# sdroh1027/DiffusionVID

Measured on AMD Instinct MI355X. Metric: frames/sec (1000x600) DiffusionVID-R101 x1, higher is better.
Workload: dtype f16

## Files before the change

### diffusionvid_amd/csrc/kernels.h

```cpp
#pragma once
#include "common.h"

struct IgemmParams {
    const half_t* in;
    const half_t* w;
    const float* bias;
    const void* res;
    void* out;
    int H, W, Cin, Ho, Wo, Cout, KH, KW, stride, pad;
    int M, Kpad, ntaps, ldc, alg_k;
    int relu, out_f32, res_mode, res_f32;
    int splitk;
    long split_stride;
    int tiles_m, tiles_n;
};
int dvid_igemm_launch(const IgemmParams& p, hipStream_t s);
int dvid_igemm2_launch(const IgemmParams& p, hipStream_t s);

bool dvid_conv3x3_halo_supported(const IgemmParams& p);
bool dvid_conv3x3_halo_preferred(const IgemmParams& p);
int dvid_conv3x3_halo_launch(const IgemmParams& p, hipStream_t s);
bool dvid_stem_pool_supported(const IgemmParams& p);
int dvid_stem_pool_launch(const IgemmParams& p, hipStream_t s);

bool dvid_wstat_supported(const IgemmParams& p);
bool dvid_wstat_preferred(const IgemmParams& p);
int dvid_wstat_launch(const IgemmParams& p, hipStream_t s);

bool dvid_bneck64_tail_preferred(int H, int W);
int dvid_bneck128_tail_launch(const half_t* t1, const half_t* w2, const float* b2, const half_t* w3, const float* b3, const half_t* res,
                              const half_t* w1n, const float* b1n, half_t* out, half_t* t1n, int n, int H, int W, hipStream_t s);
int dvid_bneck64_tail_launch(const half_t* t1, const half_t* w2, const float* b2, const half_t* w3, const float* b3, const half_t* res,
                             const half_t* ws, const float* bs, const half_t* w1n, const float* b1n, int n_next, half_t* out, half_t* t1n,
                             int n, int H, int W, hipStream_t s);

struct FrameTable {
    static constexpr int kMax = 32;
    const float* p[kMax];
};
int dvid_prep_images_launch(const float* const* frames, half_t* nhwc8, int n, int h, int w, const float* mean, const float* inv_std,
                            hipStream_t s);
int dvid_prep_images_s2d_launch(const float* const* frames, half_t* s2d16, int n, int h, int w, const float* mean, const float* inv_std,
                                hipStream_t s);
int dvid_maxpool3x3s2_launch(const half_t* in, half_t* out, int n, int h, int w, int c, hipStream_t s);
int dvid_nchw_from_nhwc_launch(const half_t* in, float* out, int n, int h, int w, int c, hipStream_t s);
int dvid_nhwc_from_nchw_launch(const float* in, half_t* out, int n, int h, int w, int c, hipStream_t s);
int dvid_add_layernorm_launch(const float* x, const float* r, const float* g, const float* b, float* y32, half_t* y16,
                              int rows, int d, int relu, hipStream_t s, int nsplit = 1, long split_stride = 0,
                              const float* xbias = nullptr);
int dvid_f32_to_f16_launch(const float* x, half_t* y, long n, hipStream_t s);
int dvid_resize_u8_launch(const unsigned char* src, int h, int w, unsigned char* tmp, float* out, int oh, int ow, int ph, int pw,
                          const int* xbounds, const int* xk, int xksize, const int* ybounds, const int* yk, int yksize, hipStream_t s);
int dvid_modulate_launch(const float* x, const float* scale, int scale_ld, const float* shift, int shift_per_row, int shift_ld,
                         half_t* y16, int rows, int rows_per_frame, int d, hipStream_t s);
int dvid_silu_f16_launch(const float* x, half_t* y, long n, hipStream_t s);

template <typename T>
struct RoiLevelsT {
    const T* feat[3];
    int h[3], w[3];
    float scale[3];
};
using RoiLevels = RoiLevelsT<half_t>;
using RoiLevels32 = RoiLevelsT<float>;
int dvid_roialign_launch(const RoiLevels& lv, int channels, const float* boxes, int n_img, int boxes_per_img, half_t* roi_out,
                         float* mean_out, hipStream_t s);

int dvid_mha_mfma_launch(const half_t* q, const half_t* k, const half_t* v, half_t* out, half_t* vt_scratch, int batch, int lq,
                         int lk, int nheads, int q_ld, int kv_ld, int out_ld, long q_bs, long kv_bs, long out_bs, hipStream_t s);

struct OutProjLnParams {
    const void* x;
    int mode;
    const half_t* wf_hi;
    const half_t* wf_lo;
    const float* w32;
    const float* wscale;
    const float* bias;
    const float* gamma;
    const float* beta;
    float* out;
    int rows, d;
    int* range_flag;
};
int dvid_outproj_ln_launch(const OutProjLnParams& p, hipStream_t s);

constexpr int SWIN_RELBIAS_PITCH = 64;
int dvid_swin_window_attn_launch(const half_t* qkv, const half_t* qkv_bias16, const float* relbias, half_t* out, int batch, int H,
                                 int W, int C, int nheads, int shift, hipStream_t s);
constexpr int SWIN12_RELBIAS_PITCH = 160;
int dvid_swin_window12_attn_launch(const half_t* qkv, const half_t* qkv_bias16, const float* relbias, half_t* out, int batch, int H,
                                   int W, int C, int nheads, int shift, hipStream_t s);
int dvid_patch_merge_ln_launch(const float* x, const float* g, const float* b, half_t* y16, int B, int H, int W, int C, hipStream_t s,
                               float* y32 = nullptr);

int dvid_dynconv_launch(const half_t* roi, const half_t* params, const float* g1, const float* b1, const float* g2,
                        const float* b2, half_t* out, int rows, hipStream_t s);
int dvid_dynconv_roi_launch(const RoiLevels& lv, int channels, const float* boxes, int n_img, int boxes_per_img, const half_t* params,
                            const float* g1, const float* b1, const float* g2, const float* b2, half_t* out, hipStream_t s);

struct HeadTailParams {
    const half_t* x16;
    const float* obj32;
    const half_t* w1f;
    const float* b1;
    const half_t* w2f;
    const float* b2;
    const float* n3g;
    const float* n3b;
    const float* scale;
    int ss_stride, rows_per_frame;
    const float* cond32;
    const half_t* wcf;
    const float* bc;
    int num_cls, num_reg, num_classes, dff;
    const half_t* clsf[4];
    const float* clsg[4];
    const float* clsb[4];
    const half_t* regf[4];
    const float* regg[4];
    const float* regb[4];
    const half_t* wlogf;
    const float* blog;
    const half_t* wdelf;
    const float* bdel;
    const float* boxes;
    float* obj_out;
    float* logits;
    float* boxes_out;
    int* bad_flag;
    long R;
    float wx, wy, ww, wh, clamp;
};
bool dvid_head_tail_supported(int hidden, int dff, int num_cls, int num_reg, int num_classes);
int dvid_head_tail_launch(const HeadTailParams& p, hipStream_t s);

int dvid_apply_deltas_launch(const float* deltas, int delta_ld, const float* boxes, float* out, int n, float wx, float wy, float ww,
                             float wh, float clamp, int* bad_flag, hipStream_t s);
int dvid_counter_normal_launch(float* out, long per_image, int n_images, uint64_t key0, hipStream_t s);
int dvid_noise_to_boxes_launch(const float* x, float* boxes, int n, float scale, float w, float h, hipStream_t s);
int dvid_topk_mask_launch(const float* logits, int n_img, int m, int c, int k1, int k2, const float* feats, int d, float* out1,
                          float* out2, hipStream_t s);

int dvid_ddim_renew_launch(const float* logits, const float* boxes, const float* xt, const float* noise, const float* fresh,
                           float* out, int n_img, int m, int c, float w, float h, float scale, float sra, float srm1, float sqrt_an,
                           float cc, float sigma, float thr, hipStream_t s);

int dvid_topk_candidates_launch(const float* logits, const float* boxes, int n_img, int nsets, int m, int c, float* cand_boxes,
                                float* cand_scores, int* cand_labels, hipStream_t s);
int dvid_topk_stream_launch(const float* logits, const float* boxes, int n_img, int nsets, int m, int c, float* cand_boxes,
                            float* cand_scores, int* cand_labels, hipStream_t s);
int dvid_nms_frames_launch(const float* cand_boxes, const float* cand_scores, const int* cand_labels, int n_img, int n, float img_w,
                           float img_h, float iou, int use_nms, int out_cap, float* out_boxes, float* out_scores, int* out_labels,
                           int* out_counts, hipStream_t s);
bool dvid_nms_frames_fits_lds(int n);
size_t dvid_nms_tiled_scratch_size(int n_img, int n);
int dvid_nms_frames_tiled_launch(const float* cand_boxes, const float* cand_scores, const int* cand_labels, int n_img, int n, float img_w,
                                 float img_h, float iou, int use_nms, int out_cap, float* out_boxes, float* out_scores, int* out_labels,
                                 int* out_counts, void* scratch, hipStream_t s);

long long dvid_seq_nms_scratch_size(const int* class_counts, const int* video_starts, int n_videos, int num_classes);
int dvid_seq_nms_launch(const float* dets, const int* counts, const int* class_counts, const int* video_starts, int n_videos, int cap, int num_classes,
                        unsigned char* keep, float* scores, int* status, void* scratch, hipStream_t s);

int dvid_cdist_launch(const float* x, int n, int d, float* dist, hipStream_t s);
int dvid_fps_launch(const float* dist, int n, int m, int bs_emul, int* idx, hipStream_t s);
int dvid_gather_rows_launch(const float* x, const int* idx, float* y, int m, int d, hipStream_t s);

struct F32GemmParams {
    const float* in;
    const float* w;
    const half_t* w_hi;
    const half_t* w_lo;
    const float* bias;
    int* range_flag;
    const float* wscale;
    const float* res;
    float* out;
    int H, W, Cin, Ho, Wo, Cout, KH, KW, stride, pad;
    int M, K, Kpad, ldc;
    int relu, res_mode;
    int tiles_m, tiles_n;
};
int dvid_f32_igemm_launch(const F32GemmParams& p, hipStream_t s);
bool dvid_f32_wstat_supported(const F32GemmParams& p);
bool dvid_f32_wstat_preferred(const F32GemmParams& p);
int dvid_f32_wstat_tile_rows(const F32GemmParams& p);
int dvid_f32_wstat_launch_tiles(const F32GemmParams& p, hipStream_t s);
bool dvid_f32_conv3x3_supported(const F32GemmParams& p);
int dvid_f32_conv3x3_launch(const F32GemmParams& p, hipStream_t s);
int dvid_f32_prep_images_launch(const float* const* frames, float* nhwc4, int n, int h, int w, const float* mean, const float* std_, hipStream_t s);
int dvid_f32_maxpool3x3s2_launch(const float* in, float* out, int n, int h, int w, int c, hipStream_t s);
int dvid_f32_silu_launch(const float* x, float* y, long n, hipStream_t s);
int dvid_f32_modulate_launch(const float* x, const float* scale, int scale_ld, const float* shift, int shift_per_row, int shift_ld, float* y,
                             int rows, int rows_per_frame, int d, hipStream_t s);
int dvid_f32_roialign_launch(const RoiLevels32& lv, int channels, const float* boxes, int n_img, int boxes_per_img, float* roi_out,
                             float* mean_out, hipStream_t s);
int dvid_f32_mha_launch(const float* q, const float* k, const float* v, float* out, int batch, int lq, int lk, int nheads, int q_ld, int kv_ld,
                        int out_ld, long q_bs, long kv_bs, long out_bs, hipStream_t s);
int dvid_f32_swin_window_attn_launch(const float* qkv, const float* qkv_bias, const float* relbias, float* out, int batch, int H, int W, int C,
                                     int nheads, int shift, hipStream_t s);
int dvid_f32_swin_window12_attn_launch(const float* qkv, const float* qkv_bias, const float* relbias, float* out, int batch, int H, int W, int C,
                                       int nheads, int shift, hipStream_t s);
int dvid_f32_dynconv_launch(const float* roi, const float* params, const float* g1, const float* b1, const float* g2, const float* b2,
                            float* out, int rows, int* range_flag, hipStream_t s);
```

### diffusionvid_amd/csrc/profile.hip

```cpp
#include <mutex>

#include "runtime.h"

bool g_prof_on = false;

namespace {
std::mutex g_prof_mu;
std::vector<ProfRec> g_prof;
std::vector<ProfRec> g_prof_pool;

int prof_take(ProfRec* r) {
    std::lock_guard<std::mutex> lock(g_prof_mu);
    if (!g_prof_pool.empty()) {
        r->a = g_prof_pool.back().a;
        r->b = g_prof_pool.back().b;
        g_prof_pool.pop_back();
        return DVID_OK;
    }
    HIP_TRY(hipEventCreate(&r->a));
    HIP_TRY(hipEventCreate(&r->b));
    return DVID_OK;
}
}

int prof_begin(ProfRec* r, hipStream_t s) {
    if (prof_take(r) != DVID_OK) return DVID_ERR_HIP;
    HIP_TRY(hipEventRecord(r->a, s));
    return DVID_OK;
}
int prof_end(const ProfRec& r, hipStream_t s) {
    HIP_TRY(hipEventRecord(r.b, s));
    std::lock_guard<std::mutex> lock(g_prof_mu);
    g_prof.push_back(r);
    return DVID_OK;
}

int igemm(const IgemmParams& p, hipStream_t s) {
    if (!g_prof_on) return dvid_igemm_launch(p, s);
    ProfRec r{.M = p.M, .N = p.Cout, .K = p.Kpad, .taps = p.ntaps, .stride = p.stride, .res_mode = p.res_mode, .family = true};
    r.flop = 2.0 * p.M * (double)p.Cout * (double)p.alg_k;
    const double in_px = (double)p.M * (p.ntaps > 1 ? p.stride * p.stride : 1);
    r.bytes = in_px * p.Cin * 2.0 + (double)p.Cout * p.Kpad * 2.0 +
              (double)p.M * p.Cout * (p.out_f32 ? 4.0 : 2.0) * (p.splitk > 1 ? p.splitk : 1) +
              (p.res_mode == 1 ? (double)p.M * p.Cout * (p.res_f32 ? 4.0 : 2.0) : p.res_mode == 2 ? (double)p.M * p.Cout * 0.5 : 0.0);
    r.kind = dvid_wstat_preferred(p) ? (p.res_mode == 1 ? "wstat2" : "wstat") : dvid_conv3x3_halo_preferred(p) ? (p.Cin == 16 ? "conv4x4_s2d" : p.Cout == 64 ? "conv3x3_c64" : "conv3x3_halo") : "igemm2";
    return prof_bracket(r, s, [&] { return dvid_igemm_launch(p, s); });
}

int bneck_tail(const half_t* t1, const half_t* w2, const float* b2, const half_t* w3, const float* b3, const half_t* res, const half_t* ws,
               const float* bs, const half_t* w1n, const float* b1n, int n_next, half_t* out, half_t* t1n, int n, int H, int W, hipStream_t s) {
    if (!g_prof_on) return dvid_bneck64_tail_launch(t1, w2, b2, w3, b3, res, ws, bs, w1n, b1n, n_next, out, t1n, n, H, W, s);
    const double M = (double)n * H * W;
    const int nn = w1n ? n_next : 0;
    const int kk = 576 + 256 + (ws ? 256 : 0) + 4 * nn;
    ProfRec r{.M = (int)M, .N = 256, .K = kk, .taps = 9, .stride = 1, .family = true};
    r.flop = 2.0 * M * 64.0 * kk;
    r.bytes = M * 2.0 * (64 + (ws ? 64 : 256) + 256 + nn) + 2.0 * 64 * kk;
    r.kind = "bneck64_tail";
    r.res_mode = ws ? 4 : 3;
    return prof_bracket(r, s, [&] { return dvid_bneck64_tail_launch(t1, w2, b2, w3, b3, res, ws, bs, w1n, b1n, n_next, out, t1n, n, H, W, s); });
}

int bneck128_tail(const half_t* t1, const half_t* w2, const float* b2, const half_t* w3, const float* b3, const half_t* res, const half_t* w1n,
                  const float* b1n, half_t* out, half_t* t1n, int n, int H, int W, hipStream_t s) {
    if (!g_prof_on) return dvid_bneck128_tail_launch(t1, w2, b2, w3, b3, res, w1n, b1n, out, t1n, n, H, W, s);
    const double M = (double)n * H * W;
    const int kk = (w2 ? 1152 : 0) + 512 + (w1n ? 512 : 0);
    ProfRec r{.M = (int)M, .N = 512, .K = kk, .taps = w2 ? 9 : 1, .stride = 1, .family = true};
    r.flop = 2.0 * M * 128.0 * kk;
    r.bytes = M * 2.0 * (128 + 512 + 512 + (w1n ? 128 : 0)) + 2.0 * 128 * kk;
    r.kind = "bneck128_tail";
    r.res_mode = 3;
    return prof_bracket(r, s, [&] { return dvid_bneck128_tail_launch(t1, w2, b2, w3, b3, res, w1n, b1n, out, t1n, n, H, W, s); });
}

extern "C" {
int dvid_profile_enable(int on) {
    g_prof_on = on != 0;
    return DVID_OK;
}
int dvid_profile_reset(void) {
    std::lock_guard<std::mutex> lock(g_prof_mu);
    for (auto& r : g_prof) g_prof_pool.push_back(r);
    g_prof.clear();
    return DVID_OK;
}
int dvid_profile_read_bytes(double* igemm_alg_bytes) {
    g_err[0] = 0;
    double b = 0;
    for (auto& r : g_prof)
        if (r.family) b += r.bytes;
    if (igemm_alg_bytes) *igemm_alg_bytes = b;
    return DVID_OK;
}

static int profile_sum(double* ms_out, double* flop_out, double* bytes_out, int64_t* n_out) {
    double ms = 0, fl = 0, by = 0;
    int64_t n = 0;
    for (auto& r : g_prof) {
        if (!r.family) continue;
        HIP_TRY(hipEventSynchronize(r.b));
        float t = 0.f;
        HIP_TRY(hipEventElapsedTime(&t, r.a, r.b));
        ms += t;
        fl += r.flop;
        by += r.bytes;
        ++n;
    }
    if (ms_out) *ms_out = ms;
    if (flop_out) *flop_out = fl;
    if (bytes_out) *bytes_out = by;
    if (n_out) *n_out = n;
    return DVID_OK;
}

int dvid_profile_read(double* igemm_ms, double* igemm_flop, int64_t* igemm_launches) {
    g_err[0] = 0;
    return profile_sum(igemm_ms, igemm_flop, nullptr, igemm_launches);
}

int dvid_profile_dump(const char* path) {
    g_err[0] = 0;
    FILE* f = fopen(path, "w");
    if (!f) FAIL(DVID_ERR_ARG, "cannot open %s", path);
    fprintf(f, "kernel,family,M,N,K,taps,stride,res_mode,ms,tflops,alg_mbytes,alg_gbs\n");
    for (auto& r : g_prof) {
        HIP_TRY(hipEventSynchronize(r.b));
        float t = 0.f;
        HIP_TRY(hipEventElapsedTime(&t, r.a, r.b));
        fprintf(f, "%s,%d,%d,%d,%d,%d,%d,%d,%.5f,%.2f,%.3f,%.1f\n", r.kind, (int)r.family, r.M, r.N, r.K, r.taps, r.stride, r.res_mode, t, r.flop / (t * 1e-3) / 1e12,
                r.bytes / 1e6, r.bytes / (t * 1e-3) / 1e9);
    }
    fclose(f);
    return DVID_OK;
}
}
```

### diffusionvid_amd/csrc/wstat.hip

```cpp
#include <stdlib.h>

#include "../../include/dvid_hip.h"
#include "common.h"
#include "kernels.h"

namespace {

__device__ __attribute__((aligned(16))) unsigned int g_zero_page_ws[4] = {0u, 0u, 0u, 0u};

typedef unsigned int uint4v __attribute__((ext_vector_type(4)));
__device__ __forceinline__ float ws_mix_add_lo(unsigned int h2, float x) {
    float d;
    asm("v_fma_mix_f32 %0, %1, 1.0, %2 op_sel_hi:[1,0,0]" : "=v"(d) : "v"(h2), "v"(x));
    return d;
}
__device__ __forceinline__ float ws_mix_add_hi(unsigned int h2, float x) {
    float d;
    asm("v_fma_mix_f32 %0, %1, 1.0, %2 op_sel:[1,0,0] op_sel_hi:[1,0,0]" : "=v"(d) : "v"(h2), "v"(x));
    return d;
}
__device__ __forceinline__ void ws_add_res8(float4v& lo, float4v& hv, half8 rv) {
    const uint4v r = __builtin_bit_cast(uint4v, rv);
    lo[0] = ws_mix_add_lo(r[0], lo[0]);
    lo[1] = ws_mix_add_hi(r[0], lo[1]);
    lo[2] = ws_mix_add_lo(r[1], lo[2]);
    lo[3] = ws_mix_add_hi(r[1], lo[3]);
    hv[0] = ws_mix_add_lo(r[2], hv[0]);
    hv[1] = ws_mix_add_hi(r[2], hv[1]);
    hv[2] = ws_mix_add_lo(r[3], hv[2]);
    hv[3] = ws_mix_add_hi(r[3], hv[3]);
}

template <int N>
__device__ __forceinline__ void ws_wait_vmcnt() {
    asm volatile("s_waitcnt vmcnt(%0)" ::"n"(N) : "memory");
}
__device__ __forceinline__ void ws_glds16(const void* gsrc, char* lds_wave_base) {
    __builtin_amdgcn_global_load_lds((const __attribute__((address_space(1))) void*)gsrc,
                                     (__attribute__((address_space(3))) void*)lds_wave_base, 16, 0, 0);
}

template <int K, int D, int TN, bool HAS_RES>
struct WsSmem {
    static constexpr int kATile = 32 * K * 2;
    static constexpr int kRTile = HAS_RES ? 8 * TN * 2048 : 0;
    static constexpr int kStage = kATile + kRTile;
    static constexpr int kBytes = D * kStage;
};

template <int K, int D, int TN, bool HAS_RES, int ACT>
__global__ __launch_bounds__(512) void wstat_kernel(IgemmParams p, int nslab) {
    constexpr bool RELU = ACT == 1;
    constexpr int NW = 8, WPX = 32;
    constexpr int SLAB = 256 * TN;
    constexpr int CH = K / 8;
    constexpr int RPP = 512 / K;
    constexpr int PIECES = 32 / RPP;
    constexpr int APW = PIECES / NW;
    constexpr int RP = HAS_RES ? 2 * TN : 0;
    constexpr int LG = APW + RP;
    constexpr int SG = 2 * TN;
    constexpr int KS = K / 16;
    constexpr int A_TILE = WsSmem<K, D, TN, HAS_RES>::kATile;
    constexpr int STAGE = WsSmem<K, D, TN, HAS_RES>::kStage;
    static_assert(PIECES % NW == 0 && APW >= 1, "every wave issues the same number of A pieces");
    static_assert((D - 2) * LG + (D - 1) * SG < 64, "vmcnt is a 6-bit counter");
    extern __shared__ __attribute__((aligned(16))) char smem[];

    const int tid = threadIdx.x;
    const int lane = tid & 63;
    const int wave = __builtin_amdgcn_readfirstlane(tid >> 6);
    const int hi = lane >> 5, lrow = lane & 31;

    const int xcd = (int)blockIdx.x & 7, q = (int)blockIdx.x >> 3;
    const int MB = p.M >> 5;
    const int xb0 = (int)((long)MB * xcd / 8), xb1 = (int)((long)MB * (xcd + 1) / 8);
    int blk0 = xb0, blk1 = xb1, slab0 = q, slab_step = WPX;
    if (nslab <= WPX) {
        const int nsub = WPX / nslab, sub = q / nslab;
        slab0 = q - sub * nslab;
        slab_step = nslab;
        blk0 = xb0 + (int)((long)(xb1 - xb0) * sub / nsub);
        blk1 = xb0 + (int)((long)(xb1 - xb0) * (sub + 1) / nsub);
        if (sub >= nsub) blk1 = blk0;
    }
    const int T = blk1 - blk0;
    if (T <= 0) return;

    const char* a_src[APW];
#pragma unroll
    for (int i = 0; i < APW; ++i) {
        const int piece = wave + NW * i;
        const int row = piece * RPP + lane / CH;
        const int lch = (lane % CH) ^ (row & 15);
        a_src[i] = reinterpret_cast<const char*>(p.in) + ((long)(blk0 * 32 + row) * K + lch * 8) * 2;
    }
    const int frag_key = lrow & 15;
    const int frag_row_off = lrow * (K * 2);

    for (int slab = slab0; slab < nslab; slab += slab_step) {
        const int n0 = slab * SLAB + 32 * TN * wave;
        half8 bf[TN][KS];
#pragma unroll
        for (int j = 0; j < TN; ++j) {
            const half_t* wrow = p.w + (long)(n0 + 32 * j + lrow) * p.Kpad + 8 * hi;
#pragma unroll
            for (int ks = 0; ks < KS; ++ks) bf[j][ks] = *reinterpret_cast<const half8*>(wrow + 16 * ks);
        }
        float bs[TN][2][8];
#pragma unroll
        for (int j = 0; j < TN; ++j)
#pragma unroll
            for (int g = 0; g < 2; ++g)
#pragma unroll
                for (int e = 0; e < 8; ++e) bs[j][g][e] = p.bias ? p.bias[n0 + 32 * j + 16 * g + 8 * hi + e] : 0.f;
        const long col = n0 + 8 * hi;
        const char* r_src = HAS_RES ? reinterpret_cast<const char*>(p.res) + ((long)(blk0 * 32 + lrow) * p.Cout + col) * 2 : nullptr;
        half_t* o_dst = reinterpret_cast<half_t*>(p.out) + (long)(blk0 * 32 + lrow) * p.ldc + col;
        const char* a_cur[APW];
#pragma unroll
        for (int i = 0; i < APW; ++i) a_cur[i] = a_src[i];

        asm volatile("s_waitcnt vmcnt(0)" ::: "memory");
#pragma unroll
        for (int j = 0; j < TN; ++j)
#pragma unroll
            for (int ks = 0; ks < KS; ++ks) asm volatile("" : "+v"(bf[j][ks]));
        __builtin_amdgcn_s_barrier();

        auto issue = [&](int ti) {
            char* const stg = smem + (ti % D) * STAGE;
            const bool more = ti + 1 < T;
#pragma unroll
            for (int i = 0; i < APW; ++i) {
                ws_glds16(a_cur[i], stg + (wave + NW * i) * 1024);
                a_cur[i] += more ? 32 * K * 2 : 0;
            }
            if (HAS_RES) {
#pragma unroll
                for (int j = 0; j < TN; ++j)
#pragma unroll
                    for (int g = 0; g < 2; ++g) ws_glds16(r_src + 64 * j + 32 * g, stg + A_TILE + ((wave * TN + j) * 2 + g) * 1024);
                r_src += more ? (long)32 * p.Cout * 2 : 0L;
            }
        };
#pragma unroll
        for (int d = 0; d < D - 1; ++d) issue(d);

        for (int t = 0; t < T; ++t) {
            ws_wait_vmcnt<(D - 2) * LG>();
            __builtin_amdgcn_s_barrier();
            asm volatile("" ::: "memory");
            issue(t + D - 1);

            const char* const stg = smem + (t % D) * STAGE;
            float16v acc[TN];
#pragma unroll
            for (int j = 0; j < TN; ++j)
#pragma unroll
                for (int r = 0; r < 16; ++r) acc[j][r] = 0.f;
#pragma unroll
            for (int ks = 0; ks < KS; ++ks) {
                const half8 fa = *reinterpret_cast<const half8*>(stg + frag_row_off + (((2 * ks + hi) ^ frag_key) * 16));
#pragma unroll
                for (int j = 0; j < TN; ++j) acc[j] = __builtin_amdgcn_mfma_f32_32x32x16_f16(bf[j][ks], fa, acc[j], 0, 0, 0);
            }
#pragma unroll
            for (int j = 0; j < TN; ++j) {
                unsigned int u[16];
#pragma unroll
                for (int r = 0; r < 16; ++r) {
                    const float f = acc[j][r];
                    u[r] = __float_as_uint(f);
                }
#pragma unroll
                for (int g = 0; g < 2; ++g)
#pragma unroll
                    for (int r = 0; r < 4; ++r) {
                        const auto sw = __builtin_amdgcn_permlane32_swap(u[8 * g + r], u[8 * g + 4 + r], false, false);
                        u[8 * g + r] = sw[0];
                        u[8 * g + 4 + r] = sw[1];
                    }
#pragma unroll
                for (int g = 0; g < 2; ++g) {
                    float4v lo, hv;
#pragma unroll
                    for (int e = 0; e < 4; ++e) {
                        lo[e] = __uint_as_float(u[8 * g + e]) + bs[j][g][e];
                        hv[e] = __uint_as_float(u[8 * g + 4 + e]) + bs[j][g][4 + e];
                    }
                    if (HAS_RES) {
                        const half8 rv = *reinterpret_cast<const half8*>(stg + A_TILE + ((wave * TN + j) * 2 + g) * 1024 + lane * 16);
                        ws_add_res8(lo, hv, rv);
                    }
                    if (ACT == 2) {
                        const float2v g0 = gelu_erf2((float2v){lo[0], lo[1]}), g1 = gelu_erf2((float2v){lo[2], lo[3]});
                        const float2v g2 = gelu_erf2((float2v){hv[0], hv[1]}), g3 = gelu_erf2((float2v){hv[2], hv[3]});
                        lo = (float4v){g0[0], g0[1], g1[0], g1[1]};
                        hv = (float4v){g2[0], g2[1], g3[0], g3[1]};
                    }
                    const half4 hlo = __builtin_convertvector(lo, half4), hhi = __builtin_convertvector(hv, half4);
                    half8 o = __builtin_shufflevector(hlo, hhi, 0, 1, 2, 3, 4, 5, 6, 7);
                    if (RELU) o = __builtin_elementwise_max(o, half8{0, 0, 0, 0, 0, 0, 0, 0});
                    *reinterpret_cast<half8*>(o_dst + 32 * j + 16 * g) = o;
                }
            }
            o_dst += (long)32 * p.ldc;
        }
        asm volatile("s_waitcnt vmcnt(0) lgkmcnt(0)" ::: "memory");
    }
}

template <int K, int D>
struct Ws2Smem {
    static constexpr int kATile = 32 * K * 2;
    static constexpr int kRTile = 32 * 256 * 2;
    static constexpr int kStage = kATile + kRTile;
    static constexpr int kCOff = D * kStage;
    static constexpr int kBytes = kCOff + 2 * kRTile;
};

template <int K, int D, bool HAS_RES, bool RELU>
__global__ __launch_bounds__(512) void wstat2_kernel(IgemmParams p, int nslab) {
    constexpr int NW = 8, WPX = 32, SLAB = 256;
    constexpr int CH = K / 8;
    constexpr int RPP = 512 / K;
    constexpr int PIECES = 32 / RPP;
    constexpr int APW = PIECES / NW;
    constexpr int RP = HAS_RES ? 2 : 0;
    constexpr int LG = APW + RP;
    constexpr int KS = K / 16;
    constexpr int A_TILE = Ws2Smem<K, D>::kATile;
    constexpr int R_TILE = Ws2Smem<K, D>::kRTile;
    constexpr int STAGE = Ws2Smem<K, D>::kStage;
    static_assert(PIECES % NW == 0 && APW >= 1, "every wave issues the same number of A pieces");
    static_assert((D - 2) * LG + (D - 1) * 2 < 64, "vmcnt is a 6-bit counter");
    extern __shared__ __attribute__((aligned(16))) char smem[];
    char* const c_img = smem + Ws2Smem<K, D>::kCOff;

    const int tid = threadIdx.x;
    const int lane = tid & 63;
    const int wave = __builtin_amdgcn_readfirstlane(tid >> 6);
    const int hi = lane >> 5, lrow = lane & 31;
    const char* const zero = reinterpret_cast<const char*>(g_zero_page_ws);

    const int xcd = (int)blockIdx.x & 7, q = (int)blockIdx.x >> 3;
    const int MB = (p.M + 31) >> 5;
    const int xb0 = (int)((long)MB * xcd / 8), xb1 = (int)((long)MB * (xcd + 1) / 8);
    int blk0 = xb0, blk1 = xb1, slab0 = q, slab_step = WPX;
    if (nslab <= WPX) {
        const int nsub = WPX / nslab, sub = q / nslab;
        slab0 = q - sub * nslab;
        slab_step = nslab;
        blk0 = xb0 + (int)((long)(xb1 - xb0) * sub / nsub);
        blk1 = xb0 + (int)((long)(xb1 - xb0) * (sub + 1) / nsub);
        if (sub >= nsub) blk1 = blk0;
    }
    const int T = blk1 - blk0;
    if (T <= 0) return;

    const char* a_src[APW];
    int a_rowm[APW];
#pragma unroll
    for (int i = 0; i < APW; ++i) {
        const int piece = wave + NW * i;
        const int row = piece * RPP + lane / CH;
        const int lch = (lane % CH) ^ (row & 15);
        a_rowm[i] = blk0 * 32 + row;
        a_src[i] = reinterpret_cast<const char*>(p.in) + ((long)a_rowm[i] * K + lch * 8) * 2;
    }
    const int frag_key = lrow & 15;
    const int frag_row_off = lrow * (K * 2);
    int rc_row[2], rc_lch[2];
#pragma unroll
    for (int i = 0; i < 2; ++i) {
        rc_row[i] = 2 * (wave + NW * i) + hi;
        rc_lch[i] = lrow ^ (rc_row[i] & 15);
    }
    int acc_off[2];
#pragma unroll
    for (int g = 0; g < 2; ++g) acc_off[g] = lrow * 512 + (((4 * wave + 2 * g + hi) ^ frag_key) * 16);

    for (int slab = slab0; slab < nslab; slab += slab_step) {
        const int n0 = slab * SLAB + 32 * wave;
        half8 bf[KS];
        {
            const half_t* wrow = p.w + (long)(n0 + lrow) * p.Kpad + 8 * hi;
#pragma unroll
            for (int ks = 0; ks < KS; ++ks) bf[ks] = *reinterpret_cast<const half8*>(wrow + 16 * ks);
        }
        float bs[2][8];
#pragma unroll
        for (int g = 0; g < 2; ++g)
#pragma unroll
            for (int e = 0; e < 8; ++e) bs[g][e] = p.bias ? p.bias[n0 + 16 * g + 8 * hi + e] : 0.f;
        const char* r_src[2];
        half_t* o_dst[2];
#pragma unroll
        for (int i = 0; i < 2; ++i) {
            const long row = (long)blk0 * 32 + rc_row[i];
            const long col = (long)slab * SLAB + rc_lch[i] * 8;
            r_src[i] = HAS_RES ? reinterpret_cast<const char*>(p.res) + (row * p.Cout + col) * 2 : zero;
            o_dst[i] = reinterpret_cast<half_t*>(p.out) + row * p.ldc + col;
        }
        const char* a_cur[APW];
#pragma unroll
        for (int i = 0; i < APW; ++i) a_cur[i] = a_src[i];

        asm volatile("s_waitcnt vmcnt(0)" ::: "memory");
#pragma unroll
        for (int ks = 0; ks < KS; ++ks) asm volatile("" : "+v"(bf[ks]));
        __builtin_amdgcn_s_barrier();

        auto issue = [&](int ti) {
            char* const stg = smem + (ti % D) * STAGE;
            const bool more = ti + 1 < T;
#pragma unroll
            for (int i = 0; i < APW; ++i) {
                ws_glds16(a_cur[i], stg + (wave + NW * i) * 1024);
                a_cur[i] += more ? 32 * K * 2 : 0;
            }
            if (HAS_RES) {
#pragma unroll
                for (int i = 0; i < 2; ++i) {
                    ws_glds16(r_src[i], stg + A_TILE + (wave + NW * i) * 1024);
                    r_src[i] += more ? (long)32 * p.Cout * 2 : 0L;
                }
            }
        };
        auto store_tile = [&](int ti) {
            const char* img = c_img + (ti & 1) * R_TILE;
#pragma unroll
            for (int i = 0; i < 2; ++i) {
                const half8 o = *reinterpret_cast<const half8*>(img + (wave + NW * i) * 1024 + lane * 16);
                *reinterpret_cast<half8*>(o_dst[i]) = o;
                o_dst[i] += (long)32 * p.ldc;
            }
        };
#pragma unroll
        for (int d = 0; d < D - 1; ++d) issue(d);

        for (int t = 0; t < T; ++t) {
            ws_wait_vmcnt<(D - 2) * LG>();
            asm volatile("s_waitcnt lgkmcnt(0)" ::: "memory");
            __builtin_amdgcn_s_barrier();
            asm volatile("" ::: "memory");
            issue(t + D - 1);
            if (t) store_tile(t - 1);

            const char* const stg = smem + (t % D) * STAGE;
            float16v acc;
#pragma unroll
            for (int r = 0; r < 16; ++r) acc[r] = 0.f;
#pragma unroll
            for (int ks = 0; ks < KS; ++ks) {
                const half8 fa = *reinterpret_cast<const half8*>(stg + frag_row_off + (((2 * ks + hi) ^ frag_key) * 16));
                acc = __builtin_amdgcn_mfma_f32_32x32x16_f16(bf[ks], fa, acc, 0, 0, 0);
            }
            unsigned int u[16];
#pragma unroll
            for (int r = 0; r < 16; ++r) {
                const float f = acc[r];
                u[r] = __float_as_uint(f);
            }
#pragma unroll
            for (int g = 0; g < 2; ++g)
#pragma unroll
                for (int r = 0; r < 4; ++r) {
                    const auto sw = __builtin_amdgcn_permlane32_swap(u[8 * g + r], u[8 * g + 4 + r], false, false);
                    u[8 * g + r] = sw[0];
                    u[8 * g + 4 + r] = sw[1];
                }
            char* const img = c_img + (t & 1) * R_TILE;
#pragma unroll
            for (int g = 0; g < 2; ++g) {
                float4v lo, hv;
#pragma unroll
                for (int e = 0; e < 4; ++e) {
                    lo[e] = __uint_as_float(u[8 * g + e]) + bs[g][e];
                    hv[e] = __uint_as_float(u[8 * g + 4 + e]) + bs[g][4 + e];
                }
                if (HAS_RES) {
                    const half8 rv = *reinterpret_cast<const half8*>(stg + A_TILE + acc_off[g]);
                    ws_add_res8(lo, hv, rv);
                }
                const half4 hlo = __builtin_convertvector(lo, half4), hhi = __builtin_convertvector(hv, half4);
                half8 o = __builtin_shufflevector(hlo, hhi, 0, 1, 2, 3, 4, 5, 6, 7);
                if (RELU) o = __builtin_elementwise_max(o, half8{0, 0, 0, 0, 0, 0, 0, 0});
                *reinterpret_cast<half8*>(img + acc_off[g]) = o;
            }
        }
        asm volatile("s_waitcnt lgkmcnt(0)" ::: "memory");
        __builtin_amdgcn_s_barrier();
        asm volatile("" ::: "memory");
        store_tile(T - 1);
        asm volatile("s_waitcnt vmcnt(0) lgkmcnt(0)" ::: "memory");
    }
}

template <int K, int D, bool HAS_RES, bool RELU>
int ws2_launch_k(const IgemmParams& p, hipStream_t s) {
    constexpr int smem = Ws2Smem<K, D>::kBytes;
    static_assert(smem <= 160 * 1024, "LDS");
    static std::atomic<unsigned long long> attr_set{0};
    if (const int rc = allow_dynamic_lds(&wstat2_kernel<K, D, HAS_RES, RELU>, smem, attr_set); rc != DVID_OK) return rc;
    hipLaunchKernelGGL((wstat2_kernel<K, D, HAS_RES, RELU>), dim3(256), dim3(512), smem, s, p, p.Cout / 256);
    LAUNCH_CHECK();
    return DVID_OK;
}

template <int K, int D>
int ws2_launch_v(const IgemmParams& p, hipStream_t s) {
    const bool res = p.res_mode == 1, relu = p.relu == 1;
    if (res) return relu ? ws2_launch_k<K, D, true, true>(p, s) : ws2_launch_k<K, D, true, false>(p, s);
    return relu ? ws2_launch_k<K, D, false, true>(p, s) : ws2_launch_k<K, D, false, false>(p, s);
}

template <int K, int D, int TN, bool HAS_RES, int RELU>
int ws_launch_k(const IgemmParams& p, hipStream_t s) {
    constexpr int smem = WsSmem<K, D, TN, HAS_RES>::kBytes;
    static_assert(smem <= 160 * 1024, "LDS");
    static std::atomic<unsigned long long> attr_set{0};
    if (const int rc = allow_dynamic_lds(&wstat_kernel<K, D, TN, HAS_RES, RELU>, smem, attr_set); rc != DVID_OK) return rc;
    hipLaunchKernelGGL((wstat_kernel<K, D, TN, HAS_RES, RELU>), dim3(256), dim3(512), smem, s, p, p.Cout / (256 * TN));
    LAUNCH_CHECK();
    return DVID_OK;
}

template <int K, int D, int TN>
int ws_launch_v(const IgemmParams& p, hipStream_t s) {
    const bool res = p.res_mode == 1, relu = p.relu == 1;
    if constexpr (TN == 1 && K <= 256) {
        if (res) return relu ? ws_launch_k<K, D, TN, true, 1>(p, s) : ws_launch_k<K, D, TN, true, 0>(p, s);
    }
    if (res) return DVID_ERR_UNSUPPORTED;
    if (p.relu == 2) return ws_launch_k<K, D, TN, false, 2>(p, s);
    return relu ? ws_launch_k<K, D, TN, false, 1>(p, s) : ws_launch_k<K, D, TN, false, 0>(p, s);
}

}

bool dvid_wstat_supported(const IgemmParams& p) {
    if (p.ntaps != 1 || p.pad != 0 || p.stride != 1 || p.Ho != p.H || p.Wo != p.W) return false;
    if (p.Cin != p.Kpad || (p.Kpad != 128 && p.Kpad != 256 && !(p.Kpad == 512 && p.res_mode == 0))) return false;
    if (p.Cout % 256) return false;
    const int ns = p.Cout / 256;
    if (!(ns <= 32 ? (32 % ns == 0 || ns == 3 || ns == 6) : ns % 32 == 0)) return false;
    if (p.out_f32 || p.splitk > 1 || p.relu > 2 || (p.ldc & 7)) return false;
    if (p.res_mode > 1 || (p.res_mode == 1 && p.res_f32)) return false;
    if (p.relu == 2 && p.res_mode) return false;
    return true;
}

bool dvid_wstat_preferred(const IgemmParams& p) {
    if (!dvid_wstat_supported(p)) return false;
    constexpr int kMinBlocks = 8;
    const int ns = p.Cout / 256;
    const long blocks_per_xcd = ((long)p.M + 31) / 32 / 8;
    const long per_wg = ns <= 32 ? blocks_per_xcd / (32 / ns) : blocks_per_xcd;
    return per_wg >= kMinBlocks;
}

static int wstat_launch_rows32(const IgemmParams& p, hipStream_t s);

int dvid_wstat_launch(const IgemmParams& p, hipStream_t s) {
    if (!dvid_wstat_supported(p)) return DVID_ERR_UNSUPPORTED;
    const int m0 = p.M & ~31, rem = p.M - m0;
    if (m0) {
        IgemmParams q = p;
        q.M = m0;
        const int rc = wstat_launch_rows32(q, s);
        if (rc != DVID_OK) return rc;
    }
    if (rem) {
        IgemmParams q = p;
        q.M = rem;
        q.in = p.in + (long)m0 * p.Kpad;
        q.out = reinterpret_cast<half_t*>(p.out) + (long)m0 * p.ldc;
        if (p.res) q.res = reinterpret_cast<const half_t*>(p.res) + (long)m0 * p.Cout;
        return dvid_igemm2_launch(q, s);
    }
    return DVID_OK;
}

static int wstat_launch_rows32(const IgemmParams& p, hipStream_t s) {
    if (p.Kpad != 512 && p.res_mode == 1) return p.Kpad == 128 ? ws2_launch_v<128, 4>(p, s) : ws2_launch_v<256, 3>(p, s);
    const int ns2 = p.Cout / 512;
    const bool wide = p.res_mode == 0 && p.Cout % 512 == 0 && ns2 >= 32 && ns2 % 32 == 0;
    if (p.Kpad == 512) return ws_launch_v<512, 4, 1>(p, s);
    if (p.Kpad == 128) return wide ? ws_launch_v<128, 6, 2>(p, s) : ws_launch_v<128, 6, 1>(p, s);
    return wide ? ws_launch_v<256, 4, 2>(p, s) : ws_launch_v<256, 4, 1>(p, s);
}
```

Baseline: 2354.

## Extend weight-stationary 1x1 GEMM to stride-2 convs and K=512 residual

Adds a strided addressing mode to the weight-stationary 1x1 kernel so stride-2 1x1 convolutions (downsample/projection layers with K=256/512) read every other input pixel directly instead of falling back to the generic igemm path. Also routes K=512 layers with a residual add through the weight-stationary kernel using a 3-stage pipeline. The intent is to move more ResNet-101 1x1 convs onto the faster weight-stationary kernel. The strided path requires Wo divisible by 32 and rejects leftover rows, so coverage depends on the feature map shapes.

```diff
diff --git a/diffusionvid_amd/csrc/kernels.h b/diffusionvid_amd/csrc/kernels.h
--- a/diffusionvid_amd/csrc/kernels.h
+++ b/diffusionvid_amd/csrc/kernels.h
@@ -26,6 +26,7 @@
 bool dvid_wstat_supported(const IgemmParams& p);
 bool dvid_wstat_preferred(const IgemmParams& p);
 int dvid_wstat_launch(const IgemmParams& p, hipStream_t s);
+const char* dvid_wstat_kernel_name(const IgemmParams& p);
 
 bool dvid_bneck64_tail_preferred(int H, int W);
 int dvid_bneck128_tail_launch(const half_t* t1, const half_t* w2, const float* b2, const half_t* w3, const float* b3, const half_t* res,
diff --git a/diffusionvid_amd/csrc/profile.hip b/diffusionvid_amd/csrc/profile.hip
--- a/diffusionvid_amd/csrc/profile.hip
+++ b/diffusionvid_amd/csrc/profile.hip
@@ -43,7 +43,7 @@
     r.bytes = in_px * p.Cin * 2.0 + (double)p.Cout * p.Kpad * 2.0 +
               (double)p.M * p.Cout * (p.out_f32 ? 4.0 : 2.0) * (p.splitk > 1 ? p.splitk : 1) +
               (p.res_mode == 1 ? (double)p.M * p.Cout * (p.res_f32 ? 4.0 : 2.0) : p.res_mode == 2 ? (double)p.M * p.Cout * 0.5 : 0.0);
-    r.kind = dvid_wstat_preferred(p) ? (p.res_mode == 1 ? "wstat2" : "wstat") : dvid_conv3x3_halo_preferred(p) ? (p.Cin == 16 ? "conv4x4_s2d" : p.Cout == 64 ? "conv3x3_c64" : "conv3x3_halo") : "igemm2";
+    r.kind = dvid_wstat_preferred(p) ? dvid_wstat_kernel_name(p) : dvid_conv3x3_halo_preferred(p) ? (p.Cin == 16 ? "conv4x4_s2d" : p.Cout == 64 ? "conv3x3_c64" : "conv3x3_halo") : "igemm2";
     return prof_bracket(r, s, [&] { return dvid_igemm_launch(p, s); });
 }
 
diff --git a/diffusionvid_amd/csrc/wstat.hip b/diffusionvid_amd/csrc/wstat.hip
--- a/diffusionvid_amd/csrc/wstat.hip
+++ b/diffusionvid_amd/csrc/wstat.hip
@@ -48,8 +48,9 @@
     static constexpr int kBytes = D * kStage;
 };
 
-template <int K, int D, int TN, bool HAS_RES, int ACT>
+template <int K, int D, int TN, bool HAS_RES, int ACT, bool S2 = false>
 __global__ __launch_bounds__(512) void wstat_kernel(IgemmParams p, int nslab) {
+    static_assert(!S2 || !HAS_RES, "the strided form has no residual ring");
     constexpr bool RELU = ACT == 1;
     constexpr int NW = 8, WPX = 32;
     constexpr int SLAB = 256 * TN;
@@ -93,10 +94,21 @@
         const int piece = wave + NW * i;
         const int row = piece * RPP + lane / CH;
         const int lch = (lane % CH) ^ (row & 15);
-        a_src[i] = reinterpret_cast<const char*>(p.in) + ((long)(blk0 * 32 + row) * K + lch * 8) * 2;
+        a_src[i] = reinterpret_cast<const char*>(p.in) + (S2 ? (long)(2 * row * K + lch * 8) * 2 : ((long)(blk0 * 32 + row) * K + lch * 8) * 2);
     }
     const int frag_key = lrow & 15;
     const int frag_row_off = lrow * (K * 2);
+    int s2_wt = 1, s2_xt0 = 0, s2_oy0 = 0;
+    long s2_base0 = 0, s2_row_adv = 0, s2_img_adv = 0;
+    if constexpr (S2) {
+        s2_wt = p.Wo >> 5;
+        const int orow = blk0 / s2_wt, img = orow / p.Ho;
+        s2_xt0 = blk0 - orow * s2_wt;
+        s2_oy0 = orow - img * p.Ho;
+        s2_base0 = ((long)(img * p.H + 2 * s2_oy0) * p.W + 64 * s2_xt0) * (K * 2);
+        s2_row_adv = (long)(2 * p.W - 2 * p.Wo) * (K * 2);
+        s2_img_adv = (long)(p.H - 2 * p.Ho) * p.W * (K * 2);
+    }
 
     for (int slab = slab0; slab < nslab; slab += slab_step) {
         const int n0 = slab * SLAB + 32 * TN * wave;
@@ -120,6 +132,8 @@
         const char* a_cur[APW];
 #pragma unroll
         for (int i = 0; i < APW; ++i) a_cur[i] = a_src[i];
+        int s2_xt = s2_xt0, s2_oy = s2_oy0;
+        long s2_base = s2_base0;
 
         asm volatile("s_waitcnt vmcnt(0)" ::: "memory");
 #pragma unroll
@@ -131,10 +145,26 @@
         auto issue = [&](int ti) {
             char* const stg = smem + (ti % D) * STAGE;
             const bool more = ti + 1 < T;
-#pragma unroll
-            for (int i = 0; i < APW; ++i) {
-                ws_glds16(a_cur[i], stg + (wave + NW * i) * 1024);
-                a_cur[i] += more ? 32 * K * 2 : 0;
+            if constexpr (S2) {
+#pragma unroll
+                for (int i = 0; i < APW; ++i) ws_glds16(a_cur[i] + s2_base, stg + (wave + NW * i) * 1024);
+                if (more) {
+                    s2_base += 64 * K * 2;
+                    if (++s2_xt == s2_wt) {
+                        s2_xt = 0;
+                        s2_base += s2_row_adv;
+                        if (++s2_oy == p.Ho) {
+                            s2_oy = 0;
+                            s2_base += s2_img_adv;
+                        }
+                    }
+                }
+            } else {
+#pragma unroll
+                for (int i = 0; i < APW; ++i) {
+                    ws_glds16(a_cur[i], stg + (wave + NW * i) * 1024);
+                    a_cur[i] += more ? 32 * K * 2 : 0;
+                }
             }
             if (HAS_RES) {
 #pragma unroll
@@ -416,13 +446,13 @@
     return relu ? ws2_launch_k<K, D, false, true>(p, s) : ws2_launch_k<K, D, false, false>(p, s);
 }
 
-template <int K, int D, int TN, bool HAS_RES, int RELU>
+template <int K, int D, int TN, bool HAS_RES, int RELU, bool S2 = false>
 int ws_launch_k(const IgemmParams& p, hipStream_t s) {
     constexpr int smem = WsSmem<K, D, TN, HAS_RES>::kBytes;
     static_assert(smem <= 160 * 1024, "LDS");
     static std::atomic<unsigned long long> attr_set{0};
-    if (const int rc = allow_dynamic_lds(&wstat_kernel<K, D, TN, HAS_RES, RELU>, smem, attr_set); rc != DVID_OK) return rc;
-    hipLaunchKernelGGL((wstat_kernel<K, D, TN, HAS_RES, RELU>), dim3(256), dim3(512), smem, s, p, p.Cout / (256 * TN));
+    if (const int rc = allow_dynamic_lds(&wstat_kernel<K, D, TN, HAS_RES, RELU, S2>, smem, attr_set); rc != DVID_OK) return rc;
+    hipLaunchKernelGGL((wstat_kernel<K, D, TN, HAS_RES, RELU, S2>), dim3(256), dim3(512), smem, s, p, p.Cout / (256 * TN));
     LAUNCH_CHECK();
     return DVID_OK;
 }
@@ -438,11 +468,27 @@
     return relu ? ws_launch_k<K, D, TN, false, 1>(p, s) : ws_launch_k<K, D, TN, false, 0>(p, s);
 }
 
+int ws_launch_res512(const IgemmParams& p, hipStream_t s) {
+    return p.relu == 1 ? ws_launch_k<512, 3, 1, true, 1>(p, s) : ws_launch_k<512, 3, 1, true, 0>(p, s);
+}
+
+template <int K>
+int ws_launch_s2(const IgemmParams& p, hipStream_t s) {
+    return p.relu == 1 ? ws_launch_k<K, 4, 1, false, 1, true>(p, s) : ws_launch_k<K, 4, 1, false, 0, true>(p, s);
+}
+
+bool ws_strided(const IgemmParams& p) {
+    return p.ntaps == 1 && p.pad == 0 && p.stride == 2 && p.Ho == (p.H - 1) / 2 + 1 && p.Wo == (p.W - 1) / 2 + 1 && p.Wo % 32 == 0 && p.Ho > 0 &&
+           p.M % (p.Ho * p.Wo) == 0;
+}
+
 }
 
 bool dvid_wstat_supported(const IgemmParams& p) {
-    if (p.ntaps != 1 || p.pad != 0 || p.stride != 1 || p.Ho != p.H || p.Wo != p.W) return false;
-    if (p.Cin != p.Kpad || (p.Kpad != 128 && p.Kpad != 256 && !(p.Kpad == 512 && p.res_mode == 0))) return false;
+    if (p.ntaps != 1 || p.pad != 0) return false;
+    if (p.stride == 1 ? (p.Ho != p.H || p.Wo != p.W) : !ws_strided(p)) return false;
+    if (p.stride != 1 && ((p.Kpad != 256 && p.Kpad != 512) || p.res_mode != 0 || p.relu > 1)) return false;
+    if (p.Cin != p.Kpad || (p.Kpad != 128 && p.Kpad != 256 && p.Kpad != 512)) return false;
     if (p.Cout % 256) return false;
     const int ns = p.Cout / 256;
     if (!(ns <= 32 ? (32 % ns == 0 || ns == 3 || ns == 6) : ns % 32 == 0)) return false;
@@ -463,9 +509,12 @@
 
 static int wstat_launch_rows32(const IgemmParams& p, hipStream_t s);
 
+const char* dvid_wstat_kernel_name(const IgemmParams& p) { return p.stride == 1 && p.Kpad != 512 && p.res_mode == 1 ? "wstat2" : "wstat"; }
+
 int dvid_wstat_launch(const IgemmParams& p, hipStream_t s) {
     if (!dvid_wstat_supported(p)) return DVID_ERR_UNSUPPORTED;
     const int m0 = p.M & ~31, rem = p.M - m0;
+    if (p.stride != 1 && rem) return DVID_ERR_ARG;
     if (m0) {
         IgemmParams q = p;
         q.M = m0;
@@ -484,6 +533,8 @@
 }
 
 static int wstat_launch_rows32(const IgemmParams& p, hipStream_t s) {
+    if (p.stride == 2) return p.Kpad == 512 ? ws_launch_s2<512>(p, s) : ws_launch_s2<256>(p, s);
+    if (p.Kpad == 512 && p.res_mode == 1) return ws_launch_res512(p, s);
     if (p.Kpad != 512 && p.res_mode == 1) return p.Kpad == 128 ? ws2_launch_v<128, 4>(p, s) : ws2_launch_v<256, 3>(p, s);
     const int ns2 = p.Cout / 512;
     const bool wide = p.res_mode == 0 && p.Cout % 512 == 0 && ns2 >= 32 && ns2 % 32 == 0;
```

After: 2390 (median of 6 runs). 1.02x the previous value.
